# creare-com/pydem

Hardware: AMD Instinct MI355X
Metric: Mcells/s (slope+aspect+UCA+TWI end-to-end) per tile; % HBM roofline (higher is better)
Workload: dtype f64

## Files before the change

pydem_amd/csrc/uca.hip:

```cpp
#include "uca_graph.h"
#include <algorithm>
#include <vector>
#include <math.h>
#include <stdlib.h>
#include <string.h>

#define PI_D 3.141592653589793

namespace {

__global__ __launch_bounds__(256) void k_section_proportion(const double *__restrict__ dir,
                                                            const uint8_t *__restrict__ flats,
                                                            const double *__restrict__ sec_theta, int64_t NN, int n, int m,
                                                            const double *__restrict__ elev,
                                                            int8_t *__restrict__ section, double *__restrict__ prop,
                                                            uint32_t *__restrict__ cinfo)
{
    (void)NN;
    for (int i = blockIdx.y; i < n; i += gridDim.y)
    for (int j = blockIdx.x * blockDim.x + threadIdx.x; j < m; j += gridDim.x * blockDim.x) {
        const int64_t c = (int64_t)i * m + j;
        const double theta = sec_theta[i];
        const double d = dir[c];
        int sec0 = (int)(int8_t)(int)floor(d / PI_D * 2.0);
// ... 387 lines not shown
            const int32_t q = base + threadIdx.x;
            const bool active = q < nq;
            QE qe; qe.c = 0; qe.cw = 0;
            if (active) qe = qc[q];
            auto push = [&](int32_t t, uint32_t ct) {
                const int32_t slot = atomicAdd(&s_next, 1);
                if (slot < A.qcap) { QE e; e.c = t; e.cw = ct; qn[slot] = e; }
                else atomicAdd(A.err, 1);
            };
            process_cell<true>(A, active, qe, (uint32_t)r, [&](bool pred, int32_t t, uint32_t ct) { if (pred) push(t, ct); }, push);
        }
        __syncthreads();
        done += nq; rounds++;
        nq = s_next;
        r++;
        __syncthreads();
    }
    if (threadIdx.x == 0) {
        cnt3[r % 3] = nq; cnt3[(r + 1) % 3] = 0; cnt3[(r + 2) % 3] = 0;
        atomicAdd(total, done); atomicAdd(total + 2, rounds);
        state[0] = r;
    }
}

#endif

#ifndef PYDEM_TH
#define PYDEM_TH 32
#endif
constexpr int TT = 32;
constexpr int TH = PYDEM_TH, HH = TH + 2;
static_assert(TH == 32 || TH == 64, "tile height");
constexpr uint32_t SP_STATE_SHIFT = 14, SP_BLOCKED = 1u << 13;
#ifndef PYDEM_STG_B
#define PYDEM_STG_B 4
#endif
constexpr int TILE_RING = TH == 32 ? 256 : 512;

struct TileW {
    uint32_t cs[TH * TT];
    union {
        unsigned long long fin[HH];
        double a0[TH];
    };
    uint16_t list[TILE_RING];
    int tail;
    int limit;
};

__device__ __forceinline__ uint16_t &sp_of(TileW &L, int idx) { return reinterpret_cast<uint16_t *>(L.cs)[2 * idx]; }
__device__ __forceinline__ uint32_t sp_state(const TileW &L, int idx) { return (L.cs[idx] >> SP_STATE_SHIFT) & 3u; }

__device__ __forceinline__ uint32_t sp_dec(TileW &L, int idx) { return atomicSub(&L.cs[idx], 1u) & 0xFFFFu; }

__device__ __forceinline__ void tile_wave_sync()
{
    __builtin_amdgcn_fence(__ATOMIC_SEQ_CST, "workgroup");
    __builtin_amdgcn_wave_barrier();
}

__device__ __forceinline__ void tile_lds_sync()
{
    __builtin_amdgcn_fence(__ATOMIC_RELEASE, "workgroup", "local");
    __builtin_amdgcn_wave_barrier();
    __builtin_amdgcn_fence(__ATOMIC_ACQUIRE, "workgroup", "local");
}

constexpr int TILE_PEND = 48;
struct TileNext {
// ... 21 lines not shown
    B.org = (int32_t)org;
    B.cinfo = reinterpret_cast<const char *>(A.cinfo) + org * 4;
    B.area = reinterpret_cast<const char *>(A.area) + org * 8;
    B.contrib = reinterpret_cast<const char *>(A.contrib) + org * 16;
    B.prop = reinterpret_cast<const char *>(A.prop) + org * 8;
    B.todo = reinterpret_cast<const char *>(A.todo_work) + org;
    return B;
}
template <typename T>
__device__ __forceinline__ T ld_off(const char *base, uint32_t off) { return *reinterpret_cast<const T *>(base + (size_t)off); }
template <typename T>
__device__ __forceinline__ void st_off(const char *base, uint32_t off, T v) { *reinterpret_cast<T *>(const_cast<char *>(base) + (size_t)off) = v; }
__device__ __forceinline__ uint32_t halo_cell(int li, int lj, int m) { return __umul24((uint32_t)li, (uint32_t)m) + (uint32_t)lj; }

__device__ __forceinline__ void fill_nbr16(int32_t *nbr16, int m)
{
    if (threadIdx.x < 8) {
        const int d = threadIdx.x, q = d + (d >> 2), di = q / 3, dj = q - 3 * di;
        nbr16[d] = ((di - 1) * m + (dj - 1)) * 16 + (((0x5A >> d) & 1) ? 0 : 8);
    }
}
__device__ __forceinline__ double in_edge_h(const TileBase &B, const int32_t *nbr16, uint32_t h, int d)
{
#ifdef PYDEM_EXP_AREAONLY
    const uint32_t off16 = h * 16u + (uint32_t)nbr16[d];
    const uint32_t uo = (off16 >> 4) * 8u;
    const double ua = ld_off<double>(B.area, uo), up = ld_off<double>(B.prop, uo);
    return (off16 & 8u) ? ua * (1 - up) : ua * up;
#else
    return ld_off<double>(B.contrib, h * 16u + (uint32_t)nbr16[d]);
#endif
}

__device__ __forceinline__ void tile_stage(const SweepArgs &A, const TileBase &B, TileW &L, uint32_t pass, int i0, int j0, int lane,
                                           uint32_t *hw = nullptr)
{
    const int n = A.n, m = A.m;
    const int half = lane >> 5, l32 = lane & 31;
    constexpr int NSET = TH * TT / 64;
    auto stage_word = [&](int gi, int gj) -> uint32_t {
        return (gi >= 0 && gi < n && gj >= 0 && gj < m) ? A.cinfo[(int64_t)gi * m + gj] : 0xFFFFFFFFu;
    };
    auto final_before = [&](uint32_t w) -> bool {
        if (w == 0xFFFFFFFFu) return true;
        const uint32_t lv = ci_level(w);
        return lv >= 1 && lv < pass;
    };
    unsigned long long colL, colR;
    {
        const uint32_t wr = stage_word(half ? i0 + TH : i0 - 1, j0 + l32);
        uint32_t wk = 0xFFFFFFFFu;
        if (lane < 4) wk = stage_word((lane & 2) ? i0 + TH : i0 - 1, (lane & 1) ? j0 + TT : j0 - 1);
        if (hw) {
            hw[(half ? TT + 2 : 0) + l32 + 1] = wr;
            if (lane < 4) hw[((lane & 2) ? TT + 2 : 0) + ((lane & 1) ? TT + 1 : 0)] = wk;
        }
        if (TH == 32) {
            const uint32_t wc = stage_word(i0 + l32, half ? j0 + TT : j0 - 1);
            if (hw) hw[2 * (TT + 2) + (half ? TH : 0) + l32] = wc;
            const unsigned long long bc = __ballot(final_before(wc));
            colL = bc & 0xFFFFFFFFull; colR = bc >> 32;
        } else {
            const uint32_t wl = stage_word(i0 + lane, j0 - 1), wq = stage_word(i0 + lane, j0 + TT);
            colL = __ballot(final_before(wl)); colR = __ballot(final_before(wq));
        }
        const bool fr = final_before(wr), fk = lane < 4 && final_before(wk);
        const unsigned long long br = __ballot(fr), bk = __ballot(fk);
        if (lane == 0) {
            L.fin[0] = ((br & 0xFFFFFFFFull) << 1) | (bk & 1ull) | (((bk >> 1) & 1ull) << 33);
            L.fin[HH - 1] = ((br >> 32) << 1) | ((bk >> 2) & 1ull) | (((bk >> 3) & 1ull) << 33);
        }
    }
    constexpr int STG_B = PYDEM_STG_B;
#pragma unroll 1
    for (int kb = 0; kb < NSET; kb += STG_B) {
        uint32_t wst[STG_B];
#pragma unroll
        for (int k = 0; k < STG_B; k++) wst[k] = stage_word(i0 + 2 * (kb + k) + half, j0 + l32);
#pragma unroll
        for (int k = 0; k < STG_B; k++) {
            const int r = 2 * (kb + k);
            const bool f = final_before(wst[k]);
            L.cs[lane + 64 * (kb + k)] = ((wst[k] == 0xFFFFFFFFu ? 0u : (wst[k] & CI_STATIC_MASK)) << 16) | ((f ? 1u : 0u) << SP_STATE_SHIFT);
            const unsigned long long b = __ballot(f);
            if (lane == 0) {
                L.fin[r + 1] = ((b & 0xFFFFFFFFull) << 1) | ((colL >> r) & 1ull) | (((colR >> r) & 1ull) << 33);
                L.fin[r + 2] = ((b >> 32) << 1) | ((colL >> (r + 1)) & 1ull) | (((colR >> (r + 1)) & 1ull) << 33);
            }
        }
    }
}

template <bool LISTED, bool WT = false>
__device__ __forceinline__ void sweep_one_tile(const SweepArgs &A, TileW &L, uint32_t pass, int tiles_x, int tid, int lane,
                                               uint8_t *__restrict__ tile_done, int32_t &n_final, const TileNext &N,
                                               int32_t *pend, int &npend, const int32_t *nbr16)
{
    const int by = tid / tiles_x, bx = tid - by * tiles_x;
    const int i0 = by * TH, j0 = bx * TT, n = A.n, m = A.m;
    const TileBase B = tile_base(A, i0, j0);
    const int half = lane >> 5, l32 = lane & 31;
    auto push_ready = [&](int cell, int consumed) {
        const int slot = atomicAdd(&L.tail, 1);
        if (slot - consumed < TILE_RING) L.list[slot % TILE_RING] = (uint16_t)cell;
        else atomicMin(&L.limit, slot);
    };
#ifdef PYDEM_TILE_PROF
    const bool prof = (A.dbg & 4) != 0 && (int)pass >= (A.dbg >> 8);
#else
    constexpr bool prof = false;
#endif
    long long tk0 = 0, tk1 = 0, tk2 = 0, tk3 = 0;
    int nrounds = 0;
    if (prof) tk0 = wall_clock64();
    if (lane == 0) { L.tail = 0; L.limit = INT32_MAX; }
    const double a0_row = (!WT && lane < TH && i0 + lane < n) ? A.a0[i0 + lane] : 0.0;
    constexpr int NSET = TH * TT / 64;
    tile_stage(A, B, L, pass, i0, j0, lane);
    tile_wave_sync();
    if (prof) tk1 = wall_clock64();
    uint32_t pitmask = 0;
    int32_t n_open = 0;
#pragma unroll 2
    for (int k = 0; k < NSET; k++) {
        const int li = 2 * k + half + 1, idx = lane + 64 * k;
        const uint32_t w = L.cs[idx];
        if (!((w >> SP_STATE_SHIFT) & 3u)) {
            const unsigned long long f0 = L.fin[li - 1], f1 = L.fin[li], f2 = L.fin[li + 1];
            const uint32_t nf = ((uint32_t)(f0 >> l32) & 7u) | (((uint32_t)(f1 >> l32) & 1u) << 3) |
                                (((uint32_t)(f1 >> (l32 + 2)) & 1u) << 4) | (((uint32_t)(f2 >> l32) & 7u) << 5);
            const uint32_t pend = __popc((w >> 16) & 0xFFu & ~nf);
            sp_of(L, idx) = (uint16_t)pend;
            n_open++;
            if (w & (CI_PIT_IN << 16)) pitmask |= 1u << k;
            else if (pend == 0) push_ready(lane + 64 * k, 0);
        }
    }
    if (pitmask) {
        constexpr int PB = 4;
#pragma unroll 1
        for (int kb = 0; kb < NSET; kb += PB) {
            if (!((pitmask >> kb) & ((1u << PB) - 1u))) continue;
            int32_t e0[PB];
#pragma unroll
            for (int k = 0; k < PB; k++) {
                e0[k] = 0;
                if (pitmask & (1u << (kb + k))) {
                    const int cell = lane + 64 * (kb + k);
                    e0[k] = ld_off<int2>(B.area, halo_cell((cell >> 5) + 1, (cell & 31) + 1, m) * 8u).x;
                }
            }
#pragma unroll
            for (int k = 0; k < PB; k++) {
// ... 111 lines not shown
                            const int q = (li - ti + 1) * 3 + (lj - tj + 1);
                            next = tcell; nd = q - (q > 4 ? 1 : 0); nv = share;
                        } else push_ready(tcell, head);
                    }
                } else if (LISTED) {
                    const int dti = ti < 1 ? -1 : (ti > TH ? 1 : 0), dtj = tj < 1 ? -1 : (tj > TT ? 1 : 0);
                    if (ti >= 1 - TH && ti <= 2 * TH && tj >= 1 - TT && tj <= 2 * TT) wake |= 1u << ((dti + 1) * 3 + dtj + 1);
                    else {
                        const int tt = ((i0 + ti - 1) / TH) * tiles_x + (j0 + tj - 1) / TT;
                        if (atomicExch(&N.flag[tt], (int32_t)pass + 1) != (int32_t)pass + 1) N.list[atomicAdd(N.count, 1)] = tt;
                    }
                }
            };
            const int sct = ci_section(cw);
            if (cw & CI_OUT1) release(li + fe1r(sct), lj + fe1c(sct), o.x, true);
            if (cw & CI_OUT2) release(li + fe2r(sct), lj + fe2c(sct), o.y, true);
            if (cw & CI_PIT_OUT)
                for (int32_t e = po.y; e < A.n_pit && A.pit_src[e] == c; e++) {
                    const int32_t dc = A.pit_dst[e];
                    const int ti = dc / m - i0 + 1, tj = dc % m - j0 + 1;
                    release(ti, tj, 0.0, false);
                }
        }
        mycell = next; cd = nd; cv = nv;
        tile_wave_sync();
    }
    if (prof) tk3 = wall_clock64();
    if (!LISTED)
        for (int k = 0; k < NSET; k++) {
            const int li = 2 * k + half + 1, idx = lane + 64 * k;
            const uint32_t w = L.cs[idx];
            if (((w >> SP_STATE_SHIFT) & 3u) == 2u) A.cinfo[(int64_t)(i0 + li - 1) * m + j0 + l32] = ci_with_level(w >> 16, pass);
        }
    for (int off = 32; off > 0; off >>= 1) { finalized += __shfl_down(finalized, off); n_open += __shfl_down(n_open, off); }
    if (LISTED) {
        for (int off = 32; off > 0; off >>= 1) wake |= __shfl_xor(wake, off);
        bool win = false;
        int tt = 0;
        if (lane < 9 && ((wake >> lane) & 1u)) { tt = tid + (lane / 3 - 1) * tiles_x + (lane % 3 - 1); win = true; }
        if (lane == 9 && L.limit != INT32_MAX) { tt = tid; win = true; }
        if (win) win = atomicExch(&N.flag[tt], (int32_t)pass + 1) != (int32_t)pass + 1;
        const unsigned long long bw = __ballot(win);
        if (win) pend[npend + __popcll(bw & ((1ull << lane) - 1ull))] = tt;
        npend += __popcll(bw);
    }
    if (lane == 0) {
        n_final += finalized;
        if (finalized == n_open) tile_done[tid] = 1;
        A.tile_open[tid] = n_open - finalized;
        if (prof) {
            const long long tk4 = wall_clock64();
            unsigned long long *acc = reinterpret_cast<unsigned long long *>(A.err + (CS_TILE_PROF - CS_QUEUE_ERR));
            atomicAdd(acc + 0, (unsigned long long)(tk1 - tk0)); atomicAdd(acc + 1, (unsigned long long)(tk2 - tk1));
            atomicAdd(acc + 2, (unsigned long long)(tk3 - tk2)); atomicAdd(acc + 3, (unsigned long long)(tk4 - tk3));
            atomicAdd(acc + 4, (unsigned long long)nrounds); atomicAdd(acc + 5, 1ull);
            if (finalized == 0) atomicAdd(acc + 6, 1ull);
        }
    }
    tile_wave_sync();
}

#include "uca_sym.inl"

#ifndef PYDEM_SWEEP_STEAL
#define PYDEM_SWEEP_STEAL 1
#endif
#ifndef PYDEM_FULL_WPB
#define PYDEM_FULL_WPB 4
#endif
constexpr int FWPB = PYDEM_FULL_WPB;
template <bool LISTED, bool WT = false>
__global__ __launch_bounds__(64 * FWPB, 32 / FWPB) void k_sweep_tiles(SweepArgs A, uint32_t pass, int tiles_x, int tiles_total,
                                                     uint8_t *__restrict__ tile_done, int32_t *n_final, TileNext N, int32_t *work8)
{
    __shared__ TileW L[FWPB];
    __shared__ int32_t s_pend[FWPB][TILE_PEND];
    __shared__ int32_t s_nbr16[8];
    fill_nbr16(s_nbr16, A.m);
    __syncthreads();
    const int wave = __builtin_amdgcn_readfirstlane(threadIdx.x >> 6), lane = threadIdx.x & 63;
    int32_t fin = 0;
    int npend = 0;
    auto flush = [&]() {
        tile_wave_sync();
        int32_t base = 0;
        if (lane == 0) base = atomicAdd(N.count, npend);
        base = __shfl(base, 0);
        if (lane < npend) N.list[base + lane] = s_pend[wave][lane];
        npend = 0;
        tile_wave_sync();
    };
#ifdef PYDEM_SWEEP_STATIC
// ... 30 lines not shown
#define PYDEM_LISTED_WPB 2
#endif
constexpr int LWPB = PYDEM_LISTED_WPB;
template <bool WT = false>
__global__ __launch_bounds__(64 * LWPB, PYDEM_LISTED_OCC) void k_sweep_tiles_listed(SweepArgs A, uint32_t pass, int tiles_x, const int32_t *__restrict__ list_in,
                                                            const int32_t *n_in, uint8_t *__restrict__ tile_done, int32_t *n_final,
                                                            TileNext N, int32_t *clear_count, int32_t *work3, SymArgs Y)
{
    __shared__ TileW L[LWPB];
    __shared__ SymLight SL[LWPB];
    const int wave = threadIdx.x >> 6, lane = threadIdx.x & 63;
    const int32_t nt = *n_in;
#ifdef PYDEM_LISTED_DYNAMIC
    if (blockIdx.x == 0 && threadIdx.x < 8) work3[((pass + 1) % 3) * 8 + threadIdx.x] = 0;
#endif
    if (blockIdx.x == 0 && threadIdx.x == 0) *clear_count = 0;
    __shared__ int32_t s_pend[LWPB][TILE_PEND];
    __shared__ int32_t s_nbr16[8];
    fill_nbr16(s_nbr16, A.m);
    __syncthreads();
    int32_t fin = 0;
    int npend = 0;
    auto flush = [&]() {
        tile_wave_sync();
        int32_t base = 0;
        if (lane == 0) base = atomicAdd(N.count, npend);
        base = __shfl(base, 0);
        if (lane < npend) N.list[base + lane] = s_pend[wave][lane];
        npend = 0;
        tile_wave_sync();
    };
#ifndef PYDEM_LISTED_DYNAMIC
    (void)work3;
    for (int32_t k = __builtin_amdgcn_readfirstlane(blockIdx.x * LWPB + wave); k < nt; k += gridDim.x * LWPB) {
#else
    const int xcd = blockIdx.x & 7;
    const int32_t per = (nt + 7) >> 3;
    int32_t *wk = &work3[(pass % 3) * 8 + xcd];
    for (;;) {
        int32_t k = 0;
        if (lane == 0) k = atomicAdd(wk, 1);
        k = __builtin_amdgcn_readfirstlane(__shfl(k, 0));
        (void)per;
        k = k * 8 + xcd;
        if (k >= nt) break;
#endif
        const int tid = __builtin_amdgcn_readfirstlane(list_in[k]);
        const uint32_t blk = Y.tile_sym ? __builtin_amdgcn_readfirstlane(Y.tile_sym[tid]) : SYM_NONE;
        if (blk != SYM_NONE) sym_light_visit<WT>(A, Y, SL[wave], pass, tiles_x, tid, lane, blk, fin, N, s_pend[wave], npend);
        else sweep_one_tile<true, WT>(A, L[wave], pass, tiles_x, tid, lane, tile_done, fin, N, s_pend[wave], npend, s_nbr16);
        if (npend > TILE_PEND - 10) flush();
    }
    if (npend) flush();
    if (lane == 0 && fin) atomicAdd(n_final, fin);
}

constexpr int DENSE_BAND = 64;
__global__ __launch_bounds__(256) void k_sweep_dense_level(SweepArgs A, uint32_t p, int32_t *n_final)
{
    const int n = A.n, m = A.m;
    int32_t fin = 0;
    const int j = blockIdx.x * blockDim.x + threadIdx.x;
    const int i_end = min(n, (int)(blockIdx.y + 1) * DENSE_BAND);
    if (j < m)
    for (int i = blockIdx.y * DENSE_BAND; i < i_end; i++) {
        const int32_t c = i * m + j;
        const uint32_t w = A.cinfo[c];
        const uint32_t lv = ci_level(w);
        if (lv >= 1 && lv != CI_LEVEL_INF) continue;
        const uint32_t cw = w & CI_STATIC_MASK;
        bool ready = true;
#pragma unroll
        for (int d = 0; d < 8; d++)
            if (cw & (1u << d)) {
                const uint32_t lu = ci_level(A.cinfo[c + NB_DI[d] * m + NB_DJ[d]]);
                ready = ready && lu >= 1 && lu < p;
            }
        if (!ready) continue;
        int2 po = make_int2(0, 0);
        if (cw & CI_PIT_IN) {
            po = pit_stash(A, c);
            for (int32_t e = po.x; e < A.n_pit && A.pin_dst[e] == c; e++) {
                const uint32_t lu = ci_level(A.cinfo[A.pin_src[e]]);
                ready = ready && lu >= 1 && lu < p;
            }
// ... 34 lines not shown

constexpr int RCAP = 256;
constexpr uint32_t RS_TAINT = 1u << 19, RS_FIN = 1u << 20;
constexpr int RS_OPEN_SHIFT = 11, RS_FINAL_SHIFT = 21;
constexpr uint32_t RS_CELL = (1u << RS_OPEN_SHIFT) - 1u, RS_CELL_OPEN = (1u << 19) - 1u;

struct TileR {
    TileW W;
    uint16_t map[TH * TT];
    double Kd[RCAP];
    double Pd[RCAP];
    uint32_t sm[RCAP];
};

__device__ __forceinline__ int nb_local(int cell, int d)
{
    const int q = d + (d >> 2);
    const int di = (q * 11) >> 5;
    return cell + (di - 1) * TT + (q - 3 * di - 1);
}

template <bool WT = false>
__device__ __forceinline__ void sweep_tile_resident(const SweepArgs &A, TileR &R, uint32_t pass, int tiles_x, int tid, int lane,
                                                    uint8_t *__restrict__ tile_done, int32_t &n_final, const TileNext &N,
                                                    int32_t *pend, int &npend)
{
    TileW &L = R.W;
    const int by = tid / tiles_x, bx = tid - by * tiles_x;
    const int i0 = by * TH, j0 = bx * TT, n = A.n, m = A.m;
    const int half = lane >> 5, l32 = lane & 31;
    constexpr int NSET = TH * TT / 64;
    if (lane == 0) L.tail = 0;
    const double a0_row = (!WT && lane < TH && i0 + lane < n) ? A.a0[i0 + lane] : 0.0;
    tile_stage(A, tile_base(A, i0, j0), L, pass, i0, j0, lane);
    tile_wave_sync();
    uint32_t pitmask = 0;
    int nslot = 0;
#pragma unroll 2
    for (int k = 0; k < NSET; k++) {
        const int li = 2 * k + half + 1, idx = lane + 64 * k;
        const uint32_t w = L.cs[idx];
        const bool open = !((w >> SP_STATE_SHIFT) & 3u);
        const unsigned long long bo = __ballot(open);
        if (open) {
            const unsigned long long f0 = L.fin[li - 1], f1 = L.fin[li], f2 = L.fin[li + 1];
            const uint32_t nf = ((uint32_t)(f0 >> l32) & 7u) | (((uint32_t)(f1 >> l32) & 1u) << 3) |
                                (((uint32_t)(f1 >> (l32 + 2)) & 1u) << 4) | (((uint32_t)(f2 >> l32) & 7u) << 5);
            const uint32_t im = (w >> 16) & 0xFFu;
            const uint32_t cnt = __popc(im & ~nf);
            sp_of(L, idx) = (uint16_t)cnt;
            const int s = nslot + __popcll(bo & ((1ull << lane) - 1ull));
            R.map[idx] = (uint16_t)s;
            R.sm[s] = (uint32_t)idx | ((im & ~nf) << RS_OPEN_SHIFT) | ((im & nf) << RS_FINAL_SHIFT);
            if (w & (CI_PIT_IN << 16)) pitmask |= 1u << k;
            else if (cnt == 0) L.list[atomicAdd(&L.tail, 1)] = (uint16_t)s;
        }
        nslot += __popcll(bo);
    }
    if (pitmask) {
#pragma unroll 1
        for (int k = 0; k < NSET; k++) {
            if (!(pitmask & (1u << k))) continue;
            const int cell = lane + 64 * k;
            const int32_t c = (i0 + (cell >> 5)) * m + j0 + (cell & 31);
            uint32_t cnt = sp_of(L, cell);
            for (int32_t e = pit_stash(A, c).x; e < A.n_pit && A.pin_dst[e] == c; e++) {
                const int32_t sc = A.pin_src[e];
// ... 747 lines not shown
    const size_t scratch_need = tiles_pad * (1 + 4 + 4 + 4 + 4 + 4) + 64 * sizeof(int32_t);
    PYDEM_TRY(tile_reserve(t, &t->scratch, &t->scratch_bytes, scratch_need, scratch_need, false));
    uint8_t *tile_done = (uint8_t *)t->scratch;
    int32_t *tile_flag = (int32_t *)(tile_done + tiles_pad);
    int32_t *tile_list[2] = {tile_flag + tiles_pad, tile_flag + 2 * tiles_pad};
    int32_t *cntT = t->counters + CS_TILE_LIST;
    A.tile_open = tile_flag + 3 * tiles_pad;
    static int64_t sym_switch = -1;
    if (sym_switch < 0) { const char *e = getenv("PYDEM_SWEEP_SYM"); sym_switch = e ? atoll(e) : 4096; if (sym_switch < 0) sym_switch = 0; }
    SymArgs Y;
    memset(&Y, 0, sizeof(Y));
    int32_t *symc = tile_flag + 4 * tiles_pad + tiles_pad;
    const bool sym_on = sym_switch > 0 && TH == 32 && t->NN / 2 < ((int64_t)1 << 31);
    if (sym_on) {
        Y.pool0 = (double *)t->queue[0]; Y.pool1 = (double *)t->queue[1];
        Y.nreg = t->NN >= ((int64_t)1 << 22) ? 16 : 2;
        Y.reg_cap = (uint32_t)((t->NN / 2) / (Y.nreg / 2));
        Y.ctr = symc; Y.tile_sym = (uint32_t *)(tile_flag + 4 * tiles_pad); Y.stat = symc + 32;
        HIP_TRY(hipMemsetAsync(Y.tile_sym, 0xff, tiles_pad * 4, t->stream));
        HIP_TRY(hipMemsetAsync(symc, 0, 64 * sizeof(int32_t), t->stream));
    }
    HIP_TRY(hipMemsetAsync(tile_done, 0, tiles_pad * 5, t->stream));
    HIP_TRY(hipMemsetAsync(A.tile_open, 0x7f, tiles_pad * 4, t->stream));
    HIP_TRY(hipMemsetAsync(cntT, 0, 4 * sizeof(int32_t), t->stream));
    if (A.dbg & 4) HIP_TRY(hipMemsetAsync(t->counters + CS_TILE_PROF, 0, CS_TILE_PROF_WORDS * sizeof(int32_t), t->stream));
    int64_t launches = 0;
    uint32_t pass = 0;
    int32_t *work16 = t->counters + CS_WORK, *work3 = t->counters + CS_WORK;
    HIP_TRY(hipMemsetAsync(work16, 0, 16 * sizeof(int32_t), t->stream));
    static int lds_pad = -1;
    if (lds_pad < 0) { const char *e = getenv("PYDEM_TILE_LDS_PAD"); lds_pad = e ? atoi(e) : 0; }
    static int res_switch = -1;
    if (res_switch < 0) { const char *e = getenv("PYDEM_SWEEP_RESIDENT"); res_switch = e ? atoi(e) : 4096; }
    int64_t listed_left = 0;
    auto run_listed = [&](int p, int64_t ntiles, int64_t stop_at) -> int {
        TileNext N;
        N.flag = tile_flag;
        listed_left = ntiles;
        while (ntiles > stop_at) {
            static int dbg_each = -1;
            if (dbg_each < 0) { const char *e = getenv("PYDEM_SWEEP_DEBUG"); dbg_each = (e && atoi(e) >= 2) ? 1 : 0; }
            const int batch = dbg_each ? 1 : ntiles < 2048 ? 16 : 8;
#ifndef PYDEM_LISTED_DYNAMIC
            const int grid = (int)(ntiles < 8192 ? (ntiles > 64 ? ntiles : 64) : 8192) * (4 / LWPB);
#else
            const int64_t want = cdiv(ntiles, 4);
            const int grid = (int)(want < 256 * PYDEM_LISTED_OCC ? (want > 16 ? want : 16) : 256 * PYDEM_LISTED_OCC);
#endif
            const bool resident = ntiles <= res_switch;
            for (int b = 0; b < batch; b++, p++) {
                N.list = tile_list[(p + 1) % 2]; N.count = &cntT[(p + 1) % 3];
                if (resident)
                    hipLaunchKernelGGL(HIP_KERNEL_NAME(k_sweep_tiles_resident<WT>), dim3((unsigned)(ntiles > 256 ? ntiles : 256)), dim3(64), 0, t->stream, A, (uint32_t)p, tiles_x,
                                       (const int32_t *)tile_list[p % 2], (const int32_t *)&cntT[p % 3], tile_done, total, N,
                                       &cntT[(p + 2) % 3], Y);
                else
                    hipLaunchKernelGGL(HIP_KERNEL_NAME(k_sweep_tiles_listed<WT>), dim3(grid), dim3(64 * LWPB), (size_t)lds_pad, t->stream, A, (uint32_t)p, tiles_x,
                                       (const int32_t *)tile_list[p % 2], (const int32_t *)&cntT[p % 3], tile_done, total, N,
                                       &cntT[(p + 2) % 3], work3, Y);
                launches++;
            }
            if (hipMemcpyAsync(t->h_counters, t->counters, CS_END * sizeof(int32_t), hipMemcpyDeviceToHost, t->stream) != hipSuccess) return -1;
            if (hipStreamSynchronize(t->stream) != hipSuccess) return -1;
            ntiles = t->h_counters[CS_TILE_LIST + p % 3];
            listed_left = ntiles;
            if (getenv("PYDEM_SWEEP_DEBUG")) fprintf(stderr, "listed tile pass %d: %lld tiles listed next, processed %d\n", p, (long long)ntiles, t->h_counters[CS_PROCESSED]);
            if (p > (int)CI_LEVEL_INF - 256) return -2;
        }
        return p;
    };
    auto replay_unfinished = [&](uint32_t pass) -> int {
        HIP_TRY(hipMemcpyAsync(t->h_counters, t->counters, CS_END * sizeof(int32_t), hipMemcpyDeviceToHost, t->stream));
        HIP_TRY(hipStreamSynchronize(t->stream));
        if ((int64_t)t->h_counters[CS_PROCESSED] >= t->NN) return 0;
        {
            ReseedCell *U = (ReseedCell *)t->queue[0];
            const int64_t cap64 = std::min<int64_t>(t->NN * 4 / (int64_t)sizeof(ReseedCell), (int64_t)1 << 22);
            uint8_t *stf = (uint8_t *)t->queue[1];
            int32_t *rc = t->counters + CS_RESEED;
            HIP_TRY(hipMemsetAsync(rc, 0, 3 * sizeof(int32_t), t->stream));
            hipLaunchKernelGGL(k_reseed_collect, dim3(grid_for(t->NN, 4096)), dim3(256), 0, t->stream, A, U, rc, (int32_t)cap64,
                               (const double *)t->elev, rc + 1);
            HIP_TRY(hipMemcpyAsync(t->h_counters, t->counters, CS_END * sizeof(int32_t), hipMemcpyDeviceToHost, t->stream));
            HIP_TRY(hipStreamSynchronize(t->stream));
            const int64_t unfinished = (int64_t)t->h_counters[CS_RESEED];
            if (unfinished == 0) {
// ... 38 lines not shown
                HIP_TRY(hipMemcpy(dH, back.data(), (size_t)nU * sizeof(ReseedBack), hipMemcpyHostToDevice));
                hipLaunchKernelGGL(k_reseed_scatter, dim3(grid_for(nU, 1024)), dim3(256), 0, t->stream, A, (const ReseedBack *)dH, nU, pass);
                HIP_TRY(hipStreamSynchronize(t->stream));
                t->h_counters[CS_PROCESSED] += (int32_t)n_done;
                HIP_TRY(hipMemcpy(t->counters + CS_PROCESSED, t->h_counters + CS_PROCESSED, sizeof(int32_t), hipMemcpyHostToDevice));
                if (getenv("PYDEM_SWEEP_DEBUG")) fprintf(stderr, "circular drainage: %lld unfinished cells, %lld finished by the re-seed replay on the host\n", (long long)unfinished, (long long)n_done);
                return 0;
            }
            std::vector<ReseedCell> hu((size_t)unfinished);
            HIP_TRY(hipMemcpyAsync(hu.data(), U, hu.size() * sizeof(ReseedCell), hipMemcpyDeviceToHost, t->stream));
            HIP_TRY(hipStreamSynchronize(t->stream));
            std::sort(hu.begin(), hu.end(), [](const ReseedCell &a, const ReseedCell &b) { return a.c < b.c; });
            HIP_TRY(hipMemcpyAsync(U, hu.data(), hu.size() * sizeof(ReseedCell), hipMemcpyHostToDevice, t->stream));
            hipLaunchKernelGGL(HIP_KERNEL_NAME(k_reseed_replay<WT>), dim3(1), dim3(64), 0, t->stream, A, (const ReseedCell *)U, (int32_t)unfinished,
                               (const double *)t->elev, (const double *)t->pits.w, stf, stf + unfinished, t->h_counters[CS_RESEED + 1],
                               (int)opt->circular_ref_maxcount, pass, total, rc + 2);
            launches += 2;
            HIP_TRY(hipMemcpyAsync(t->h_counters, t->counters, CS_END * sizeof(int32_t), hipMemcpyDeviceToHost, t->stream));
            HIP_TRY(hipStreamSynchronize(t->stream));
            if (getenv("PYDEM_SWEEP_DEBUG")) fprintf(stderr, "circular drainage: %lld unfinished cells, %d finished by the re-seed replay\n", (long long)unfinished, t->h_counters[CS_RESEED + 2]);
        }
        return 0;
    };
#ifdef PYDEM_SWEEP_QUEUE
    static int sweep_mode = -1;
    if (sweep_mode < 0) { const char *e = getenv("PYDEM_SWEEP_MODE"); sweep_mode = (e && !strcmp(e, "queue")) ? 1 : 0; }
    if (WT && sweep_mode == 1) { pydem_set_error("pydem_uca_weighted: PYDEM_SWEEP_MODE=queue is not supported (the weighted sweep runs the tile passes)"); return -6; }
#else
    constexpr int sweep_mode = 0;
#endif
#ifdef PYDEM_SWEEP_STATIC
    const unsigned full_grid = (unsigned)(((tiles_total + 31) / 32) * 8);
#else
    const unsigned full_grid = (unsigned)std::min<int64_t>(((tiles_total + 31) / 32) * 8, 256 * (32 / FWPB));
#endif

    if (sweep_mode == 0) {
        static int first_kind = -1;
        if (first_kind < 0) { const char *e = getenv("PYDEM_SWEEP_FIRST"); first_kind = (e && !strcmp(e, "lds")) ? 1 : 0; }
        static int dense_levels = -1;
        if (dense_levels < 0) { const char *e = getenv("PYDEM_SWEEP_DENSE"); dense_levels = e ? atoi(e) : 0; if (dense_levels < 0) dense_levels = 0; }
        for (int lv = 1; !WT && lv <= dense_levels; lv++) {
            hipLaunchKernelGGL(k_sweep_dense_level, dim3((unsigned)cdiv(m, 256), (unsigned)cdiv(n, DENSE_BAND)), dim3(256), 0, t->stream,
                               A, (uint32_t)lv, total);
            launches++;
        }
        const uint32_t pb = WT ? 0u : (uint32_t)dense_levels;
        if (!WT && first_kind == 1 && TH == 32 && pb == 0)
            hipLaunchKernelGGL(k_sweep_first, dim3((unsigned)(((tiles_total + 7) / 8) * 8)), dim3(256), 0, t->stream, A, tiles_x, tiles_total, tile_done, total);
        else {
            TileNext N0; N0.flag = nullptr; N0.list = nullptr; N0.count = nullptr;
            hipLaunchKernelGGL(HIP_KERNEL_NAME(k_sweep_tiles<false, WT>), dim3(full_grid), dim3(64 * FWPB), (size_t)lds_pad, t->stream, A, pb + 1u, tiles_x, tiles_total, tile_done, total, N0, work16);
        }
        TileNext N; N.flag = tile_flag; N.list = tile_list[(pb + 3) % 2]; N.count = &cntT[(pb + 3) % 3];
        hipLaunchKernelGGL(HIP_KERNEL_NAME(k_sweep_tiles<true, WT>), dim3(full_grid), dim3(64 * FWPB), (size_t)lds_pad, t->stream, A, pb + 2u, tiles_x, tiles_total, tile_done, total, N, work16 + 8);
        HIP_TRY(hipMemsetAsync(work3, 0, CS_WORK_WORDS * sizeof(int32_t), t->stream));
        launches += 2;
        HIP_TRY(hipMemcpyAsync(t->h_counters, t->counters, CS_END * sizeof(int32_t), hipMemcpyDeviceToHost, t->stream));
        HIP_TRY(hipStreamSynchronize(t->stream));
        if (getenv("PYDEM_SWEEP_DEBUG")) fprintf(stderr, "tile passes %u-%u: %d cells of %lld, %d tiles listed\n", pb + 1, pb + 2, t->h_counters[CS_PROCESSED], (long long)t->NN, t->h_counters[CS_TILE_LIST + (pb + 3) % 3]);
        int p_end = run_listed((int)pb + 3, t->h_counters[CS_TILE_LIST + (pb + 3) % 3], sym_on ? sym_switch : 0);
        if (sym_on && p_end > 0 && listed_left > 0) {
            const uint32_t ps = (uint32_t)p_end;
            TileNext N3; N3.flag = tile_flag; N3.list = tile_list[(ps + 1) % 2]; N3.count = &cntT[(ps + 1) % 3];
            HIP_TRY(hipMemsetAsync(&cntT[(ps + 2) % 3], 0, sizeof(int32_t), t->stream));
            int32_t *cand = tile_list[ps % 2];
            hipLaunchKernelGGL(k_sym_candidates, dim3((unsigned)cdiv(tiles_total, 256)), dim3(256), 0, t->stream, (const uint8_t *)tile_done, (const int32_t *)A.tile_open,
// ... 210 lines not shown
```

pydem_amd/csrc/uca_graph.h:

```cpp
#pragma once
#include "internal.h"
#include <stdlib.h>

namespace {

constexpr uint32_t CI_OUT1 = 1u << 8, CI_OUT2 = 1u << 9, CI_PIT_OUT = 1u << 10, CI_PIT_IN = 1u << 11;
constexpr int CI_SEC_SHIFT = 12, CI_LEVEL_SHIFT = 15;
constexpr uint32_t CI_LEVEL_INF = 0x1FFFFu, CI_STATIC_MASK = 0x7FFFu;
__device__ __forceinline__ uint32_t ci_level(uint32_t w) { return w >> CI_LEVEL_SHIFT; }
__device__ __forceinline__ int ci_section(uint32_t w) { return (int)((w >> CI_SEC_SHIFT) & 7u); }
__device__ __forceinline__ uint32_t ci_with_level(uint32_t w, uint32_t lv) { return (w & CI_STATIC_MASK) | (lv << CI_LEVEL_SHIFT); }

__device__ __constant__ const int NB_DI[8] = {-1, -1, -1, 0, 0, 1, 1, 1};
__device__ __constant__ const int NB_DJ[8] = {-1, 0, 1, -1, 1, -1, 0, 1};
__device__ __constant__ const int NB_S0[8] = {6, 5, 4, 0, 3, 0, 1, 2};
__device__ __constant__ const int NB_S1[8] = {7, 6, 5, 7, 4, 1, 2, 3};

__device__ __forceinline__ bool keep_edge(double w, double z_to, double z_from)
{
    return !isnan(w) && (w > 1e-8) && (z_to <= z_from);
}

struct SweepArgs {
    uint32_t *cinfo;
    const double *prop, *a0;
    double *area;
    double2 *contrib;
    uint8_t *todo_work;
    int n, m;
    const int32_t *pit_src, *pit_dst;
    const int32_t *pin_dst, *pin_src; const double *pin_w;
    int64_t n_pit;
    int dbg;
    int32_t qcap;
    int32_t *err;
    int32_t *tile_open;
};

struct QE { int32_t c; uint32_t cw; };

enum CounterSlot : int {
    CS_FRONTIER = 0,
    CS_PROCESSED = 3,
    CS_SOURCES = 4,
    CS_ROUNDS = 5,
    CS_EDGE_REACHED = 6,
    CS_EDGE_CLEARED = 7,
    CS_EDGE_SEEDS = 8,
    CS_CASCADE_STATE = 12,
    CS_SWEEP_STATE = 14,
    CS_QUEUE_ERR = 15,
    CS_WINDOW = 16,
    CS_H_CB_TOTALS = 16,
    CS_WORK = 16, CS_WORK_WORDS = 24,
// ... 1 lines not shown
    CS_EINC_PROF = 40,
    CS_ND_COUNT = 48,
    CS_ND_NEXT = 50,
    CS_NAN_SEEDS = 53,
    CS_COND_EDGES = 54,
    CS_TILE_LIST = 56,
    CS_RESEED = 60,
    CS_FLAT_SAVE = 62,
    CS_END = 64
};
static_assert(CS_FRONTIER + 3 <= CS_PROCESSED && CS_ROUNDS == CS_PROCESSED + 2, "kernels reach the round count through the processed-cells pointer");
static_assert(CS_ROUNDS < CS_EDGE_REACHED && CS_EDGE_SEEDS < CS_CASCADE_STATE && CS_CASCADE_STATE < CS_SWEEP_STATE && CS_SWEEP_STATE < CS_QUEUE_ERR,
              "the scalars of a cascade are live together");
static_assert(CS_QUEUE_ERR < CS_WINDOW && CS_WINDOW <= CS_WORK, "one copy of the window shows the host every scalar of a cascade, and no scratch");
static_assert(CS_WORK + CS_WORK_WORDS <= CS_EINC_PROF, "zeroing the per-tile scratch leaves the fix-up's words alone");
static_assert(CS_TILE_PROF + CS_TILE_PROF_WORDS <= CS_TILE_LIST, "the visit profile ends before the tile lists");
static_assert(CS_EINC_PROF + 8 <= CS_ND_COUNT && CS_ND_COUNT + 2 <= CS_ND_NEXT && CS_ND_NEXT < CS_NAN_SEEDS && CS_NAN_SEEDS < CS_COND_EDGES
              && CS_COND_EDGES < CS_TILE_LIST, "the fix-up's words are live together and stay clear of the sweep's");
static_assert(CS_TILE_LIST + 4 <= CS_RESEED && CS_RESEED + 3 <= CS_END && CS_FLAT_SAVE + 2 <= CS_END, "the sweep's lists and replay words are live together");

inline int grid_for(int64_t work, int cap) { const int64_t g = cdiv(work, 256); return (int)(g < cap ? (g > 0 ? g : 1) : cap); }
}

static void fill_sweep_args(pydem_tile *t, SweepArgs &A)
{
    A.cinfo = t->cinfo; A.prop = t->prop; A.a0 = t->row_area; A.area = t->uca;
    A.contrib = (double2 *)t->contrib; A.todo_work = t->todo_work; A.n = (int)t->n; A.m = (int)t->m;
    A.pit_src = t->pits.src; A.pit_dst = t->pits.dst; A.n_pit = t->pits.n_edges;
    A.pin_dst = t->pits.in_dst; A.pin_src = t->pits.in_src; A.pin_w = t->pits.in_w;
    A.qcap = (int32_t)(t->NN / 2 < INT32_MAX ? t->NN / 2 : INT32_MAX);
    A.err = t->counters + CS_QUEUE_ERR;
    A.tile_open = nullptr;
    { const char *e = getenv("PYDEM_TILE_DEBUG"); A.dbg = e ? atoi(e) : 0; }
}
```

Before: 5574.

## Prefetch next tile's cinfo halo while sweeping current tile in listed sweep

In the static listed-tile sweep, each wave now loads the next tile's list entry, symmetry word and full cinfo halo/rows into registers (TileStaged) at phases inside the current tile's sweep, then commits them to LDS at the start of the next tile. This is meant to hide global-memory latency of tile staging behind the current tile's work. It raises register pressure (a full row array per lane), which may reduce occupancy. A grid-cap env knob and a pipeline-disable switch are also added.

```diff
diff --git a/pydem_amd/csrc/uca.hip b/pydem_amd/csrc/uca.hip
--- a/pydem_amd/csrc/uca.hip
+++ b/pydem_amd/csrc/uca.hip
@@ -443,9 +443,6 @@
 constexpr int TH = PYDEM_TH, HH = TH + 2;
 static_assert(TH == 32 || TH == 64, "tile height");
 constexpr uint32_t SP_STATE_SHIFT = 14, SP_BLOCKED = 1u << 13;
-#ifndef PYDEM_STG_B
-#define PYDEM_STG_B 4
-#endif
 constexpr int TILE_RING = TH == 32 ? 256 : 512;
 
 struct TileW {
@@ -533,8 +530,54 @@
 #endif
 }
 
-__device__ __forceinline__ void tile_stage(const SweepArgs &A, const TileBase &B, TileW &L, uint32_t pass, int i0, int j0, int lane,
-                                           uint32_t *hw = nullptr)
+#ifndef PYDEM_STG_B
+#define PYDEM_STG_B 4
+#endif
+struct TileStaged {
+    uint32_t wr, wk;
+    uint32_t wc, wq;
+    uint32_t row[TH * TT / 64];
+};
+__device__ __forceinline__ bool final_before(uint32_t w, uint32_t pass)
+{
+    if (w == 0xFFFFFFFFu) return true;
+    const uint32_t lv = ci_level(w);
+    return lv >= 1 && lv < pass;
+}
+__device__ __forceinline__ void tile_commit_ring(TileW &L, uint32_t pass, uint32_t wr, uint32_t wk, uint32_t wc, uint32_t wq, int lane,
+                                                 uint32_t *hw, unsigned long long &colL, unsigned long long &colR)
+{
+    const int half = lane >> 5, l32 = lane & 31;
+    if (hw) {
+        hw[(half ? TT + 2 : 0) + l32 + 1] = wr;
+        if (lane < 4) hw[((lane & 2) ? TT + 2 : 0) + ((lane & 1) ? TT + 1 : 0)] = wk;
+    }
+    if (TH == 32) {
+        if (hw) hw[2 * (TT + 2) + (half ? TH : 0) + l32] = wc;
+        const unsigned long long bc = __ballot(final_before(wc, pass));
+        colL = bc & 0xFFFFFFFFull; colR = bc >> 32;
+    } else {
+        colL = __ballot(final_before(wc, pass)); colR = __ballot(final_before(wq, pass));
+    }
+    const bool fr = final_before(wr, pass), fk = lane < 4 && final_before(wk, pass);
+    const unsigned long long br = __ballot(fr), bk = __ballot(fk);
+    if (lane == 0) {
+        L.fin[0] = ((br & 0xFFFFFFFFull) << 1) | (bk & 1ull) | (((bk >> 1) & 1ull) << 33);
+        L.fin[HH - 1] = ((br >> 32) << 1) | ((bk >> 2) & 1ull) | (((bk >> 3) & 1ull) << 33);
+    }
+}
+__device__ __forceinline__ void tile_commit_rows(TileW &L, uint32_t pass, uint32_t w, int k, int lane, unsigned long long colL, unsigned long long colR)
+{
+    const int r = 2 * k;
+    const bool f = final_before(w, pass);
+    L.cs[lane + 64 * k] = ((w == 0xFFFFFFFFu ? 0u : (w & CI_STATIC_MASK)) << 16) | ((f ? 1u : 0u) << SP_STATE_SHIFT);
+    const unsigned long long b = __ballot(f);
+    if (lane == 0) {
+        L.fin[r + 1] = ((b & 0xFFFFFFFFull) << 1) | ((colL >> r) & 1ull) | (((colR >> r) & 1ull) << 33);
+        L.fin[r + 2] = ((b >> 32) << 1) | ((colL >> (r + 1)) & 1ull) | (((colR >> (r + 1)) & 1ull) << 33);
+    }
+}
+__device__ __forceinline__ void tile_stage(const SweepArgs &A, TileW &L, uint32_t pass, int i0, int j0, int lane, uint32_t *hw = nullptr)
 {
     const int n = A.n, m = A.m;
     const int half = lane >> 5, l32 = lane & 31;
@@ -542,35 +585,15 @@
     auto stage_word = [&](int gi, int gj) -> uint32_t {
         return (gi >= 0 && gi < n && gj >= 0 && gj < m) ? A.cinfo[(int64_t)gi * m + gj] : 0xFFFFFFFFu;
     };
-    auto final_before = [&](uint32_t w) -> bool {
-        if (w == 0xFFFFFFFFu) return true;
-        const uint32_t lv = ci_level(w);
-        return lv >= 1 && lv < pass;
-    };
     unsigned long long colL, colR;
     {
         const uint32_t wr = stage_word(half ? i0 + TH : i0 - 1, j0 + l32);
         uint32_t wk = 0xFFFFFFFFu;
         if (lane < 4) wk = stage_word((lane & 2) ? i0 + TH : i0 - 1, (lane & 1) ? j0 + TT : j0 - 1);
-        if (hw) {
-            hw[(half ? TT + 2 : 0) + l32 + 1] = wr;
-            if (lane < 4) hw[((lane & 2) ? TT + 2 : 0) + ((lane & 1) ? TT + 1 : 0)] = wk;
-        }
-        if (TH == 32) {
-            const uint32_t wc = stage_word(i0 + l32, half ? j0 + TT : j0 - 1);
-            if (hw) hw[2 * (TT + 2) + (half ? TH : 0) + l32] = wc;
-            const unsigned long long bc = __ballot(final_before(wc));
-            colL = bc & 0xFFFFFFFFull; colR = bc >> 32;
-        } else {
-            const uint32_t wl = stage_word(i0 + lane, j0 - 1), wq = stage_word(i0 + lane, j0 + TT);
-            colL = __ballot(final_before(wl)); colR = __ballot(final_before(wq));
-        }
-        const bool fr = final_before(wr), fk = lane < 4 && final_before(wk);
-        const unsigned long long br = __ballot(fr), bk = __ballot(fk);
-        if (lane == 0) {
-            L.fin[0] = ((br & 0xFFFFFFFFull) << 1) | (bk & 1ull) | (((bk >> 1) & 1ull) << 33);
-            L.fin[HH - 1] = ((br >> 32) << 1) | ((bk >> 2) & 1ull) | (((bk >> 3) & 1ull) << 33);
-        }
+        uint32_t wc, wq = 0;
+        if (TH == 32) wc = stage_word(i0 + l32, half ? j0 + TT : j0 - 1);
+        else { wc = stage_word(i0 + lane, j0 - 1); wq = stage_word(i0 + lane, j0 + TT); }
+        tile_commit_ring(L, pass, wr, wk, wc, wq, lane, hw, colL, colR);
     }
     constexpr int STG_B = PYDEM_STG_B;
 #pragma unroll 1
@@ -579,23 +602,44 @@
 #pragma unroll
         for (int k = 0; k < STG_B; k++) wst[k] = stage_word(i0 + 2 * (kb + k) + half, j0 + l32);
 #pragma unroll
-        for (int k = 0; k < STG_B; k++) {
-            const int r = 2 * (kb + k);
-            const bool f = final_before(wst[k]);
-            L.cs[lane + 64 * (kb + k)] = ((wst[k] == 0xFFFFFFFFu ? 0u : (wst[k] & CI_STATIC_MASK)) << 16) | ((f ? 1u : 0u) << SP_STATE_SHIFT);
-            const unsigned long long b = __ballot(f);
-            if (lane == 0) {
-                L.fin[r + 1] = ((b & 0xFFFFFFFFull) << 1) | ((colL >> r) & 1ull) | (((colR >> r) & 1ull) << 33);
-                L.fin[r + 2] = ((b >> 32) << 1) | ((colL >> (r + 1)) & 1ull) | (((colR >> (r + 1)) & 1ull) << 33);
-            }
-        }
-    }
-}
-
-template <bool LISTED, bool WT = false>
+        for (int k = 0; k < STG_B; k++) tile_commit_rows(L, pass, wst[k], kb + k, lane, colL, colR);
+    }
+}
+__device__ __forceinline__ void tile_stage_issue(const SweepArgs &A, int i0, int j0, int lane, TileStaged &S)
+{
+    const int n = A.n, m = A.m;
+    const int half = lane >> 5, l32 = lane & 31;
+    constexpr int NSET = TH * TT / 64;
+    const char *base = reinterpret_cast<const char *>(A.cinfo) + ((int64_t)(i0 - 1) * m + (j0 - 1)) * 4;
+    auto stage_word = [&](int li, int lj) -> uint32_t {
+        const int gi = i0 - 1 + li, gj = j0 - 1 + lj;
+        return (gi >= 0 && gi < n && gj >= 0 && gj < m) ? ld_off<uint32_t>(base, halo_cell(li, lj, m) * 4u) : 0xFFFFFFFFu;
+    };
+    S.wr = stage_word(half ? TH + 1 : 0, l32 + 1);
+    S.wk = 0xFFFFFFFFu;
+    if (lane < 4) S.wk = stage_word((lane & 2) ? TH + 1 : 0, (lane & 1) ? TT + 1 : 0);
+    if (TH == 32) { S.wc = stage_word(l32 + 1, half ? TT + 1 : 0); S.wq = 0; }
+    else { S.wc = stage_word(lane + 1, 0); S.wq = stage_word(lane + 1, TT + 1); }
+    const uint32_t voff = halo_cell(half + 1, l32 + 1, m) * 4u;
+    const bool col_in = j0 + l32 < m;
+#pragma unroll
+    for (int k = 0; k < NSET; k++)
+        S.row[k] = (col_in && i0 + 2 * k + half < n) ? ld_off<uint32_t>(base + (int64_t)(2 * k) * m * 4, voff) : 0xFFFFFFFFu;
+}
+__device__ __forceinline__ void tile_stage_commit(TileW &L, uint32_t pass, const TileStaged &S, int lane)
+{
+    constexpr int NSET = TH * TT / 64;
+    unsigned long long colL, colR;
+    tile_commit_ring(L, pass, S.wr, S.wk, S.wc, S.wq, lane, nullptr, colL, colR);
+#pragma unroll
+    for (int k = 0; k < NSET; k++) tile_commit_rows(L, pass, S.row[k], k, lane, colL, colR);
+}
+struct NoAhead { __device__ __forceinline__ void operator()(int) const {} };
+
+template <bool LISTED, bool WT = false, typename Ahead>
 __device__ __forceinline__ void sweep_one_tile(const SweepArgs &A, TileW &L, uint32_t pass, int tiles_x, int tid, int lane,
                                                uint8_t *__restrict__ tile_done, int32_t &n_final, const TileNext &N,
-                                               int32_t *pend, int &npend, const int32_t *nbr16)
+                                               int32_t *pend, int &npend, const int32_t *nbr16, const TileStaged *S, Ahead &&ahead)
 {
     const int by = tid / tiles_x, bx = tid - by * tiles_x;
     const int i0 = by * TH, j0 = bx * TT, n = A.n, m = A.m;
@@ -617,9 +661,12 @@
     if (lane == 0) { L.tail = 0; L.limit = INT32_MAX; }
     const double a0_row = (!WT && lane < TH && i0 + lane < n) ? A.a0[i0 + lane] : 0.0;
     constexpr int NSET = TH * TT / 64;
-    tile_stage(A, B, L, pass, i0, j0, lane);
+    ahead(0);
+    if (S) tile_stage_commit(L, pass, *S, lane);
+    else tile_stage(A, L, pass, i0, j0, lane);
     tile_wave_sync();
     if (prof) tk1 = wall_clock64();
+    ahead(1);
     uint32_t pitmask = 0;
     int32_t n_open = 0;
 #pragma unroll 2
@@ -797,6 +844,7 @@
             const uint32_t w = L.cs[idx];
             if (((w >> SP_STATE_SHIFT) & 3u) == 2u) A.cinfo[(int64_t)(i0 + li - 1) * m + j0 + l32] = ci_with_level(w >> 16, pass);
         }
+    ahead(2);
     for (int off = 32; off > 0; off >>= 1) { finalized += __shfl_down(finalized, off); n_open += __shfl_down(n_open, off); }
     if (LISTED) {
         for (int off = 32; off > 0; off >>= 1) wake |= __shfl_xor(wake, off);
@@ -823,6 +871,13 @@
         }
     }
     tile_wave_sync();
+}
+template <bool LISTED, bool WT = false>
+__device__ __forceinline__ void sweep_one_tile(const SweepArgs &A, TileW &L, uint32_t pass, int tiles_x, int tid, int lane,
+                                               uint8_t *__restrict__ tile_done, int32_t &n_final, const TileNext &N,
+                                               int32_t *pend, int &npend, const int32_t *nbr16)
+{
+    sweep_one_tile<LISTED, WT>(A, L, pass, tiles_x, tid, lane, tile_done, n_final, N, pend, npend, nbr16, nullptr, NoAhead());
 }
 
 #include "uca_sym.inl"
@@ -919,7 +974,41 @@
     };
 #ifndef PYDEM_LISTED_DYNAMIC
     (void)work3;
-    for (int32_t k = __builtin_amdgcn_readfirstlane(blockIdx.x * LWPB + wave); k < nt; k += gridDim.x * LWPB) {
+    const bool pipe = !(A.dbg & TILE_DBG_UNPIPELINED);
+    const int32_t stride = (int32_t)(gridDim.x * LWPB);
+    auto sym_word = [&](int tile) -> uint32_t { return Y.tile_sym ? Y.tile_sym[tile] : SYM_NONE; };
+    TileStaged S = {};
+    int32_t k = __builtin_amdgcn_readfirstlane(blockIdx.x * LWPB + wave);
+    int tid = 0;
+    uint32_t blk = SYM_NONE;
+    if (k < nt) {
+        tid = __builtin_amdgcn_readfirstlane(list_in[k]);
+        blk = __builtin_amdgcn_readfirstlane(sym_word(tid));
+        if (blk == SYM_NONE) tile_stage_issue(A, (tid / tiles_x) * TH, (tid % tiles_x) * TT, lane, S);
+    }
+    for (; k < nt; k += stride) {
+        const bool more = k + stride < nt, overlap = pipe && blk == SYM_NONE;
+        TileStaged Sn = {};
+        int32_t tid_v = 0;
+        uint32_t blk_v = SYM_NONE;
+        int tid_next = 0;
+        uint32_t blk_next = SYM_NONE;
+        auto look = [&](int phase) __attribute__((always_inline)) {
+            if (!more) return;
+            if (phase == 0) tid_v = list_in[k + stride];
+            else if (phase == 1) { tid_next = __builtin_amdgcn_readfirstlane(tid_v); blk_v = sym_word(tid_next); }
+            else {
+                blk_next = __builtin_amdgcn_readfirstlane(blk_v);
+                if (blk_next == SYM_NONE) tile_stage_issue(A, (tid_next / tiles_x) * TH, (tid_next % tiles_x) * TT, lane, Sn);
+            }
+        };
+        auto ahead = [&](int phase) __attribute__((always_inline)) { if (overlap) look(phase); };
+        if (blk != SYM_NONE) sym_light_visit<WT>(A, Y, SL[wave], pass, tiles_x, tid, lane, blk, fin, N, s_pend[wave], npend);
+        else sweep_one_tile<true, WT>(A, L[wave], pass, tiles_x, tid, lane, tile_done, fin, N, s_pend[wave], npend, s_nbr16, &S, ahead);
+        if (!overlap) { look(0); look(1); look(2); }
+        if (npend > TILE_PEND - 10) flush();
+        tid = tid_next; blk = blk_next; S = Sn;
+    }
 #else
     const int xcd = blockIdx.x & 7;
     const int32_t per = (nt + 7) >> 3;
@@ -931,13 +1020,13 @@
         (void)per;
         k = k * 8 + xcd;
         if (k >= nt) break;
-#endif
         const int tid = __builtin_amdgcn_readfirstlane(list_in[k]);
         const uint32_t blk = Y.tile_sym ? __builtin_amdgcn_readfirstlane(Y.tile_sym[tid]) : SYM_NONE;
         if (blk != SYM_NONE) sym_light_visit<WT>(A, Y, SL[wave], pass, tiles_x, tid, lane, blk, fin, N, s_pend[wave], npend);
         else sweep_one_tile<true, WT>(A, L[wave], pass, tiles_x, tid, lane, tile_done, fin, N, s_pend[wave], npend, s_nbr16);
         if (npend > TILE_PEND - 10) flush();
     }
+#endif
     if (npend) flush();
     if (lane == 0 && fin) atomicAdd(n_final, fin);
 }
@@ -1038,7 +1127,7 @@
     constexpr int NSET = TH * TT / 64;
     if (lane == 0) L.tail = 0;
     const double a0_row = (!WT && lane < TH && i0 + lane < n) ? A.a0[i0 + lane] : 0.0;
-    tile_stage(A, tile_base(A, i0, j0), L, pass, i0, j0, lane);
+    tile_stage(A, L, pass, i0, j0, lane);
     tile_wave_sync();
     uint32_t pitmask = 0;
     int nslot = 0;
@@ -1852,6 +1941,8 @@
     if (lds_pad < 0) { const char *e = getenv("PYDEM_TILE_LDS_PAD"); lds_pad = e ? atoi(e) : 0; }
     static int res_switch = -1;
     if (res_switch < 0) { const char *e = getenv("PYDEM_SWEEP_RESIDENT"); res_switch = e ? atoi(e) : 4096; }
+    int64_t grid_cap = INT32_MAX;
+    { const char *e = getenv("PYDEM_SWEEP_GRID_CAP"); if (e && atoll(e) > 0) grid_cap = atoll(e); }
     int64_t listed_left = 0;
     auto run_listed = [&](int p, int64_t ntiles, int64_t stop_at) -> int {
         TileNext N;
@@ -1862,7 +1953,7 @@
             if (dbg_each < 0) { const char *e = getenv("PYDEM_SWEEP_DEBUG"); dbg_each = (e && atoi(e) >= 2) ? 1 : 0; }
             const int batch = dbg_each ? 1 : ntiles < 2048 ? 16 : 8;
 #ifndef PYDEM_LISTED_DYNAMIC
-            const int grid = (int)(ntiles < 8192 ? (ntiles > 64 ? ntiles : 64) : 8192) * (4 / LWPB);
+            const int grid = (int)std::min<int64_t>((ntiles < 8192 ? (ntiles > 64 ? ntiles : 64) : 8192) * (4 / LWPB), grid_cap);
 #else
             const int64_t want = cdiv(ntiles, 4);
             const int grid = (int)(want < 256 * PYDEM_LISTED_OCC ? (want > 16 ? want : 16) : 256 * PYDEM_LISTED_OCC);
@@ -1871,7 +1962,7 @@
             for (int b = 0; b < batch; b++, p++) {
                 N.list = tile_list[(p + 1) % 2]; N.count = &cntT[(p + 1) % 3];
                 if (resident)
-                    hipLaunchKernelGGL(HIP_KERNEL_NAME(k_sweep_tiles_resident<WT>), dim3((unsigned)(ntiles > 256 ? ntiles : 256)), dim3(64), 0, t->stream, A, (uint32_t)p, tiles_x,
+                    hipLaunchKernelGGL(HIP_KERNEL_NAME(k_sweep_tiles_resident<WT>), dim3((unsigned)std::min<int64_t>(ntiles > 256 ? ntiles : 256, grid_cap)), dim3(64), 0, t->stream, A, (uint32_t)p, tiles_x,
                                        (const int32_t *)tile_list[p % 2], (const int32_t *)&cntT[p % 3], tile_done, total, N,
                                        &cntT[(p + 2) % 3], Y);
                 else
@@ -1976,7 +2067,7 @@
 #ifdef PYDEM_SWEEP_STATIC
     const unsigned full_grid = (unsigned)(((tiles_total + 31) / 32) * 8);
 #else
-    const unsigned full_grid = (unsigned)std::min<int64_t>(((tiles_total + 31) / 32) * 8, 256 * (32 / FWPB));
+    const unsigned full_grid = (unsigned)std::min<int64_t>(std::min<int64_t>(((tiles_total + 31) / 32) * 8, 256 * (32 / FWPB)), 8 * std::min<int64_t>(grid_cap, 1 << 20));
 #endif
 
     if (sweep_mode == 0) {
diff --git a/pydem_amd/csrc/uca_graph.h b/pydem_amd/csrc/uca_graph.h
--- a/pydem_amd/csrc/uca_graph.h
+++ b/pydem_amd/csrc/uca_graph.h
@@ -20,6 +20,8 @@
 {
     return !isnan(w) && (w > 1e-8) && (z_to <= z_from);
 }
+
+constexpr int TILE_DBG_UNPIPELINED = 8;
 
 struct SweepArgs {
     uint32_t *cinfo;
@@ -87,4 +89,5 @@
     A.err = t->counters + CS_QUEUE_ERR;
     A.tile_open = nullptr;
     { const char *e = getenv("PYDEM_TILE_DEBUG"); A.dbg = e ? atoi(e) : 0; }
+    { const char *e = getenv("PYDEM_SWEEP_PIPELINE"); if (e && atoi(e) == 0) A.dbg |= TILE_DBG_UNPIPELINED; else A.dbg &= ~TILE_DBG_UNPIPELINED; }
 }
```

After: 5614, median of 6. No clear change (+0.7%).
